# Wenlin-Chen/ADKF-IFT

Hardware: AMD Instinct MI355X
Metric: meta-tasks/sec (N_support=128, d=256) (higher is better)
Workload: dtype f32

## Files before the change

adkf_ift_amd/csrc/adkf_gp.hip:

```cpp
#include <hip/hip_runtime.h>
#include <algorithm>
#include <cstdio>
#include <cstdlib>

#include "../../include/adkf_gp.h"
#include "ard.h"
#include "pna.h"
#include "readout.h"
#include "block.h"
#include "outer_step.h"
#include "refine64.h"
#include "hyper.h"
#include "large_fused.h"
#include "gemm_x3.h"
#include "dense_x3.h"
#include "predict_stream.h"
#include "thompson_stream.h"
#include "believer_stream.h"

#include "host_common.h"
#include "host_gp.h"
#include "host_ard.h"
#include "host_stream.h"

extern "C" {

const char* adkf_last_hip_error(void) { return hipGetErrorString(g_last_hip_error); }

const char* adkf_version(void) { return "adkf_gp 0.1 (gfx950)"; }

int adkf_path_info(int32_t ns_max, int32_t nq_max) {
    if (ns_max <= 0 || nq_max < 0 || ns_max > MAX_POINTS || nq_max > MAX_POINTS) return ADKF_E_SIZE;
    int bits = 0;
    const int hi = ns_max > nq_max ? ns_max : nq_max;
    if (nq_max > 0 && use_fused_outer(ns_max, nq_max)) bits |= ADKF_PATH_FUSED_OUTER;
    if (hi > REG_POINTS) { bits |= ADKF_PATH_BLOCKED; if (lg_fused_by_size(hi)) bits |= ADKF_PATH_BLOCKED_FUSED; }
    if (carve(nullptr, 1, ns_max, nq_max > 0 ? nq_max : 1, 4).w64_stride != 0) bits |= ADKF_PATH_R64_REGION;
    if (refine64_lds_optin()) bits |= ADKF_PATH_R64_LDS;
    return bits;
}

int adkf_max_points(void) { return MAX_POINTS; }

size_t adkf_workspace_bytes(int32_t T, int32_t ns_max, int32_t nq_max, int32_t d) {
    if (T <= 0 || ns_max <= 0 || nq_max < 0 || d <= 0) return 0;
    return carve(nullptr, T, ns_max, nq_max, d).bytes;
}

size_t adkf_workspace_bytes_ard(int32_t T, int32_t ns_max, int32_t nq_max, int32_t d) {
    if (T <= 0 || ns_max <= 0 || nq_max < 0 || d <= 0) return 0;
    return carve_ard(nullptr, carve(nullptr, T, ns_max, nq_max, d).bytes, T, ns_max, nq_max, d).bytes;
}

static int median_core(const adkf_batch_t* b, const Workspace& w, float* l0, const InitArgs& init, bool* fused, hipStream_t st) {
    int rc = stage_dist(b, w, has_query(b), st);
    if (rc) return rc;
    *fused = b->ns_max <= 256;
    if (b->ns_max <= 128) k_median<512, 16><<<grid_for(b->T, 1), 512, 0, st>>>(w.D2ss, b->n_s, b->ns_max, l0, b->T, init);
    else if (b->ns_max <= 256) k_median<1024, 32><<<grid_for(b->T, 1), 1024, 0, st>>>(w.D2ss, b->n_s, b->ns_max, l0, b->T, init);
    else {
        LgMedian lm{w.D2ss, b->n_s, b->ns_max, l0, b->T, reinterpret_cast<uint32_t*>(w.lg_med), w.lg_med + b->T, w.lg_med + 2 * (size_t)b->T};
        hipMemsetAsync(lm.hist, 0, sizeof(int) * 256 * (size_t)b->T, st);
        const int rows_blocks = ceil_div(b->ns_max, 16) < 64 ? ceil_div(b->ns_max, 16) : 64;
        for (int pass = 0; pass < 4; ++pass) {
            k_lg_med_hist<<<dim3(rows_blocks, b->T), 256, 0, st>>>(lm, pass);
            k_lg_med_pick<<<ceil_div(b->T, 64), 64, 0, st>>>(lm, pass);
        }
    }
    LAUNCH_OK();
    return 0;
}

int adkf_median_lengthscale(const adkf_batch_t* b, float* l0, void* ws, size_t ws_bytes, void* stream) {
    int rc = check_batch(b, false);
    if (rc) return rc;
    if (!l0 || !ws) return ADKF_E_BADARG;
    Workspace w = carve_for(b, ws);
    if (ws_bytes < w.bytes) return ADKF_E_WORKSPACE;
    bool fused;
    return median_core(b, w, l0, InitArgs{0, 0, nullptr, nullptr}, &fused, static_cast<hipStream_t>(stream));
}

int adkf_init_params(const adkf_batch_t* b, int32_t use_numeric_labels, int32_t use_lengthscale_prior, float* phi,
                     float* priors, float* l0, void* ws, size_t ws_bytes, void* stream) {
    int rc = check_batch(b, false);
    if (rc) return rc;
    if (!phi || !priors || !ws) return ADKF_E_BADARG;
    Workspace w = carve_for(b, ws);
    if (ws_bytes < w.bytes) return ADKF_E_WORKSPACE;
    float* l0p = l0 ? l0 : w.l0;
    hipStream_t st = static_cast<hipStream_t>(stream);
    InitArgs init{use_numeric_labels, use_lengthscale_prior, phi, priors};
    ArdWs a{};
    if (is_ard(b)) {
        a = carve_ard(ws, w.bytes, b->T, b->ns_max, b->nq_max, b->d);
        if (ws_bytes < a.bytes) return ADKF_E_WORKSPACE;
        init.phi = a.phi3;
    }
    bool fused = false;
    rc = median_core(b, w, l0p, init, &fused, st);
    if (rc) return rc;
    if (!fused) k_init_params<<<ceil_div(b->T, 64), 64, 0, st>>>(l0p, b->T, init);
    if (is_ard(b)) k_ard_expand_phi<<<dim3(ceil_div(2 + b->d, 256), b->T), 256, 0, st>>>(a.phi3, phi, b->T, 2 + b->d);
    LAUNCH_OK();
    return 0;
}

int adkf_mll_value_grad(const adkf_batch_t* b, const float* phi, float* f_in, float* g_phi, float* dZ_s, int32_t* info,
                        void* ws, size_t ws_bytes, void* stream) {
    int rc = check_batch(b, false);
    if (rc) return rc;
    if (!phi || !f_in || !info || !ws || !b->y_s || !b->priors) return ADKF_E_BADARG;
    if (is_ard(b)) {
        ArdCtx c;
        adkf_batch_t b0 = *b; b0.flags &= ~ADKF_BATCH_REUSE_INNER;
        rc = ard_setup(&b0, ws, ws_bytes, static_cast<hipStream_t>(stream), c);
        if (rc) return rc;
        rc = ard_eval(c, phi, f_in, g_phi ? g_phi : c.a.ge, info);
        if (rc) return rc;
        if (dZ_s) {
            ArdDzFin fs{c.v, c.a.G, nullptr, nullptr, nullptr, 0.f, dZ_s, b->n_s, c.ns};
            k_ard_dz_fin<<<dim3(ceil_div(c.d, 256), c.ns, c.T), 256, 0, c.st>>>(fs);
            LAUNCH_OK();
        }
        return 0;
    }
    Workspace w = carve_for(b, ws);
    if (ws_bytes < w.bytes) return ADKF_E_WORKSPACE;
    hipStream_t st = static_cast<hipStream_t>(stream);
    rc = stage_dist(b, w, has_query(b), st);
    if (rc) return rc;
    InnerArgs ia = inner_args(b, w, const_cast<float*>(phi), info);
    ia.f_out = f_in; ia.g_out = g_phi;
    rc = launch_inner(ia, w, st);
    if (rc) return rc;
    launch_refine(make_tv(b, w, false), b, w, false, 0, nullptr, info, st, f_in, g_phi, nullptr);
    if (dZ_s) {
        TaskView tv = make_tv(b, w, false);
        const int win_tiles = std::max(1, std::min(64, b->ns_max * b->ns_max / 2048));
        WinArgs wa{tv, w.Ainv, w.D2ss, w.Wss, w.scal, b->T, win_tiles};
        k_win<<<grid_for(b->T, win_tiles), 256, 0, st>>>(wa);
        hipMemsetAsync(dZ_s, 0, (size_t)b->T * b->ns_max * b->d * sizeof(float), st);
        ProbDZ<false> pz; pz.tv = tv; pz.Wss = w.Wss; pz.Wqs = nullptr; pz.Wqq = nullptr; pz.Zs = b->Z_s; pz.Zq = nullptr; pz.dZ = dZ_s; pz.d = b->d;
        launch_gemm(pz, b->T, b->ns_max, b->d, st, x3_for(b->d));
        LAUNCH_OK();
    }
    return 0;
}

int adkf_fit(const adkf_batch_t* b, float* phi, const adkf_fit_options_t* opt, float* f_final, float* gnorm,
             int32_t* n_evals, int32_t* info, void* ws, size_t ws_bytes, void* stream) {
    int rc = check_batch(b, false);
    if (rc) return rc;
    if (!phi || !opt || !info || !ws || !b->y_s || !b->priors || opt->max_evals < 2) return ADKF_E_BADARG;
    if (is_ard(b)) return ard_fit(b, phi, opt, f_final, gnorm, n_evals, info, ws, ws_bytes, static_cast<hipStream_t>(stream));
    Workspace w = carve_for(b, ws);
    if (ws_bytes < w.bytes) return ADKF_E_WORKSPACE;
    hipStream_t st = static_cast<hipStream_t>(stream);
    rc = stage_dist(b, w, has_query(b), st);
    if (rc) return rc;
    InnerArgs ia = inner_args(b, w, phi, info);
    ia.f_out = f_final; ia.gnorm_out = gnorm; ia.nevals_out = n_evals;
    ia.max_evals = opt->max_evals; ia.exact_evals = opt->exact_evals; ia.gtol = opt->gtol; ia.ftol = opt->ftol;
    if (opt->ev_start && hipEventRecord(static_cast<hipEvent_t>(opt->ev_start), st) != hipSuccess) return ADKF_E_LAUNCH;
    rc = launch_inner(ia, w, st);
    if (opt->ev_stop && hipEventRecord(static_cast<hipEvent_t>(opt->ev_stop), st) != hipSuccess) return ADKF_E_LAUNCH;
    if (rc) return rc;
    if (!(b->flags & ADKF_BATCH_DEFER_REFINE)) launch_refine(make_tv(b, w, false), b, w, false, 0, nullptr, info, st, f_final, nullptr, gnorm);
    LAUNCH_OK();
    return 0;
}

int adkf_predict(const adkf_batch_t* b, const float* phi, float* mean, float* var, float* cov, int32_t* info, void* ws,
                 size_t ws_bytes, void* stream) {
    int rc = check_batch(b, true);
    if (rc) return rc;
    if (!phi || !mean || !info || !ws || !b->y_s || !b->priors) return ADKF_E_BADARG;
    if (is_ard(b)) {
        ArdCtx c;
        rc = ard_setup(b, ws, ws_bytes, static_cast<hipStream_t>(stream), c);
        if (rc) return rc;
        if (b->flags & ADKF_BATCH_REUSE_INNER) k_ard_params<<<dim3(ceil_div(c.d, 256), c.T), 256, 0, c.st>>>(c.v, phi);
        rc = ard_outer(c, phi, 0, nullptr, info, false);
        if (rc) return rc;
        adkf_batch_t bq = c.bt;
        return predict_core(&bq, c.w, mean, var, cov, info, c.st);
    }
    Workspace w = carve_for(b, ws);
    if (ws_bytes < w.bytes) return ADKF_E_WORKSPACE;
    hipStream_t st = static_cast<hipStream_t>(stream);
    rc = stage_dist(b, w, true, st);
    if (rc) return rc;
    rc = inner_stage(b, w, phi, info, true, st);
    if (rc) return rc;
    return predict_core(b, w, mean, var, cov, info, st);
}

int adkf_predict_marginal(const adkf_batch_t* b, const float* phi, int32_t flags, const float* Zq, const int64_t* q_off, int64_t rows,
                          const float* best_f, float* mean, float* var, float* ei, int32_t* info, void* ws, size_t ws_bytes, void* stream) {
    return predict_marginal(false, b, phi, flags, Zq, q_off, rows, best_f, mean, var, ei, info, ws, ws_bytes, stream);
}

int adkf_predict_marginal_ard(const adkf_batch_t* b, const float* phi, int32_t flags, const float* Zq, const int64_t* q_off, int64_t rows,
                              const float* best_f, float* mean, float* var, float* ei, int32_t* info, void* ws, size_t ws_bytes, void* stream) {
    return predict_marginal(true, b, phi, flags, Zq, q_off, rows, best_f, mean, var, ei, info, ws, ws_bytes, stream);
}

size_t adkf_predict_pool_scratch_bytes(int32_t T, int32_t k) {
    if (T <= 0 || k <= 0 || k > ADKF_POOL_TOPK_MAX) return 0;
    return pool_scratch(nullptr, T, k).bytes;
}

int adkf_predict_pool(const adkf_batch_t* b, const float* phi, int32_t flags, const float* X, int64_t rows, const float* best_f,
                      const int64_t* excl_idx, const int64_t* excl_off, float* mean, float* var, float* ei, int32_t k, int64_t* top_idx,
                      float* top_val, int32_t* info, void* ws, size_t ws_bytes, void* scratch, size_t scratch_bytes, void* stream) {
    int rc = check_support_only(b, phi, info, ws, rows);
    if (rc) return rc;
    if (k < 0) return ADKF_E_BADARG;
    if (flags & ~(ADKF_PM_LATENT | ADKF_PM_MAXIMIZE | ADKF_PM_SCORE_MEAN | ADKF_PM_LOG_EI)) return ADKF_E_BADARG;
    const bool by_mean = (flags & ADKF_PM_SCORE_MEAN) != 0;
    if ((flags & ADKF_PM_LOG_EI) && !ei && (k == 0 || by_mean)) return ADKF_E_BADARG;
    if (rows > 0 && !X) return ADKF_E_BADARG;
    if ((ei || (k > 0 && !by_mean)) && !best_f) return ADKF_E_BADARG;
    if (k > 0 && (!top_idx || !top_val)) return ADKF_E_BADARG;
    if (!mean && !var && !ei && k == 0) return ADKF_E_BADARG;
    if (excl_idx && !excl_off) return ADKF_E_BADARG;
    if (k > ADKF_POOL_TOPK_MAX) return ADKF_E_SIZE;
    const PoolScratch l = pool_scratch(scratch, b->T, k);
    if ((rc = check_scratch(scratch, scratch_bytes, l.bytes))) return rc;
    PmCtx c;
    rc = pm_prepare(b, phi, info, ws, ws_bytes, stream, c);
    if (rc) return rc;
    PmPool pool = pm_pool(excl_idx, excl_off, k, b->T, l.cand_idx, l.cand_val, rows, c.st);
    pool.score_mean = by_mean ? 1 : 0; pool.top_idx = top_idx; pool.top_val = top_val;
    const PmCall io{flags & (ADKF_PM_LATENT | ADKF_PM_MAXIMIZE | ADKF_PM_LOG_EI), X, nullptr, rows, best_f, mean, var, ei, info, &pool};
    return c.ard ? pm_launch<true, true>(c, io) : pm_launch<false, true>(c, io);
}

size_t adkf_thompson_pool_scratch_bytes(int32_t T, int32_t ns_max, int32_t S, int32_t m) {
    if (T <= 0 || ns_max <= 0 || ns_max > MAX_POINTS || S < 1 || S > ADKF_TS_SAMPLES_MAX) return 0;
    if (m < 64 || m > ADKF_TS_FEATURES_MAX || (m & 63)) return 0;
    return ts_scratch(nullptr, T, ns_max, S).bytes;
}

int adkf_thompson_pool(const adkf_batch_t* b, const float* phi, int32_t flags, const float* X, int64_t rows, const float* omega,
                       const float* phase, int32_t m, const float* w, const float* eps, int32_t S, const int64_t* excl_idx,
                       const int64_t* excl_off, float* paths, int64_t* sel_idx, float* sel_val, int32_t* info, void* ws, size_t ws_bytes,
                       void* scratch, size_t scratch_bytes, void* stream) {
    return thompson_pool(false, b, phi, flags, X, rows, omega, phase, m, w, eps, S, excl_idx, excl_off, paths, sel_idx, sel_val, info, ws,
                         ws_bytes, scratch, scratch_bytes, stream);
}

int adkf_thompson_pool_ard(const adkf_batch_t* b, const float* phi, int32_t flags, const float* X, int64_t rows, const float* omega,
                           const float* phase, int32_t m, const float* w, const float* eps, int32_t S, const int64_t* excl_idx,
                           const int64_t* excl_off, float* paths, int64_t* sel_idx, float* sel_val, int32_t* info, void* ws, size_t ws_bytes,
                           void* scratch, size_t scratch_bytes, void* stream) {
    return thompson_pool(true, b, phi, flags, X, rows, omega, phase, m, w, eps, S, excl_idx, excl_off, paths, sel_idx, sel_val, info, ws,
                         ws_bytes, scratch, scratch_bytes, stream);
}

size_t adkf_believer_pool_scratch_bytes(int32_t T, int32_t ns_max, int32_t d, int32_t q) {
    if (T <= 0 || ns_max <= 0 || ns_max > MAX_POINTS || d <= 0 || q < 1 || q > ADKF_POOL_TOPK_MAX) return 0;
    return bv_scratch(nullptr, T, ns_max, d, q).bytes;
}

int adkf_believer_pool(const adkf_batch_t* b, const float* phi, int32_t flags, const float* X, int64_t rows, const float* best_f,
                       const int64_t* excl_idx, const int64_t* excl_off, int32_t q, float* trace, int64_t* sel_idx, float* sel_val,
                       float* sel_mean, float* sel_var, int32_t* info, void* ws, size_t ws_bytes, void* scratch, size_t scratch_bytes,
                       void* stream) {
    return believer_pool(false, b, phi, flags, X, rows, best_f, excl_idx, excl_off, q, trace, sel_idx, sel_val, sel_mean, sel_var, info, ws,
                         ws_bytes, scratch, scratch_bytes, stream);
}

int adkf_believer_pool_ard(const adkf_batch_t* b, const float* phi, int32_t flags, const float* X, int64_t rows, const float* best_f,
                           const int64_t* excl_idx, const int64_t* excl_off, int32_t q, float* trace, int64_t* sel_idx, float* sel_val,
                           float* sel_mean, float* sel_var, int32_t* info, void* ws, size_t ws_bytes, void* scratch, size_t scratch_bytes,
                           void* stream) {
    return believer_pool(true, b, phi, flags, X, rows, best_f, excl_idx, excl_off, q, trace, sel_idx, sel_val, sel_mean, sel_var, info, ws,
                         ws_bytes, scratch, scratch_bytes, stream);
}

int adkf_outer_nll_value_grad(const adkf_batch_t* b, const float* phi, float* f_out, float* g_phi, float* dZ_s,
                              float* dZ_q, int32_t* info, void* ws, size_t ws_bytes, void* stream) {
    int rc = check_batch(b, true);
    if (rc) return rc;
    if (!phi || !f_out || !info || !ws || !b->y_s || !b->y_q || !b->priors) return ADKF_E_BADARG;
    if (is_ard(b))
        return ard_ift(b, phi, 0, false, 0, 0.f, f_out, dZ_s, dZ_q, g_phi, nullptr, nullptr, info, ws, ws_bytes, static_cast<hipStream_t>(stream));
    Workspace w = carve_for(b, ws);
    if (ws_bytes < w.bytes) return ADKF_E_WORKSPACE;
    return outer_pipeline(b, w, phi, 0, false, f_out, dZ_s, dZ_q, g_phi, nullptr, nullptr, info, static_cast<hipStream_t>(stream));
}

int adkf_ift_hypergrad(const adkf_batch_t* b, const float* phi, int32_t flags, float* f_out, float* dZ_s, float* dZ_q,
                       float* g_phi_out, float* v, float* H, int32_t* info, void* ws, size_t ws_bytes, void* stream) {
    int rc = check_batch(b, true);
    if (rc) return rc;
    if (!phi || !f_out || !dZ_s || !dZ_q || !info || !ws || !b->y_s || !b->y_q || !b->priors) return ADKF_E_BADARG;
    if (is_ard(b)) {
        if (H) return ADKF_E_BADARG;
        return ard_ift(b, phi, flags, true, ADKF_CG_DEFAULT_MAXITER, ADKF_CG_DEFAULT_TOL, f_out, dZ_s, dZ_q, g_phi_out, v, nullptr, info,
                       ws, ws_bytes, static_cast<hipStream_t>(stream));
    }
    Workspace w = carve_for(b, ws);
    if (ws_bytes < w.bytes) return ADKF_E_WORKSPACE;
    return outer_pipeline(b, w, phi, flags, true, f_out, dZ_s, dZ_q, g_phi_out, v, H, info, static_cast<hipStream_t>(stream));
}

int adkf_double_path_tasks(const adkf_batch_t* b, int32_t* flagged, void* ws, size_t ws_bytes, void* stream) {
    int rc = check_batch(b, true);
    if (rc) return rc;
    if (!flagged || !ws || is_ard(b)) return ADKF_E_BADARG;
    Workspace w = carve_for(b, ws);
    if (ws_bytes < w.bytes) return ADKF_E_WORKSPACE;
    (void)hipGetLastError();
    k_double_path_tasks<<<ceil_div(b->T, 256), 256, 0, static_cast<hipStream_t>(stream)>>>(w.scal, b->ns_max, b->nq_max, w.w64 ? r64_threshold() : INFINITY, b->T, flagged);
    LAUNCH_OK();
    return 0;
}

int adkf_ift_hypergrad_cg(const adkf_batch_t* b, const float* phi, int32_t flags, int32_t cg_maxiter, float cg_tol, float* f_out,
                          float* dZ_s, float* dZ_q, float* g_phi_out, float* v, int32_t* cg_iters, int32_t* info, void* ws,
                          size_t ws_bytes, void* stream) {
    int rc = check_batch(b, true);
    if (rc) return rc;
    if (!is_ard(b) || cg_maxiter < 1 || !(cg_tol > 0.f)) return ADKF_E_BADARG;
    if (!phi || !f_out || !dZ_s || !dZ_q || !info || !ws || !b->y_s || !b->y_q || !b->priors) return ADKF_E_BADARG;
    return ard_ift(b, phi, flags, true, cg_maxiter, cg_tol, f_out, dZ_s, dZ_q, g_phi_out, v, cg_iters, info, ws, ws_bytes,
                   static_cast<hipStream_t>(stream));
}

int adkf_check_info(const int32_t* info, int32_t T, void* stream) {
    if (!info || T <= 0) return ADKF_E_BADARG;
    int32_t* host = static_cast<int32_t*>(malloc(sizeof(int32_t) * (size_t)T));
    if (!host) return ADKF_E_BADARG;
    hipStream_t st = static_cast<hipStream_t>(stream);
    if (hipMemcpyAsync(host, info, sizeof(int32_t) * (size_t)T, hipMemcpyDeviceToHost, st) != hipSuccess || hipStreamSynchronize(st) != hipSuccess) {
        free(host);
        return ADKF_E_LAUNCH;
    }
    int rc = 0;
    for (int t = 0; t < T; ++t) if (host[t] != 0) { rc = t + 1; break; }
    free(host);
    return rc;
}

}

#include "host_gnn.h"
#include "host_dense.h"
```

adkf_ift_amd/csrc/host_gp.h:

```cpp
#pragma once
#include "host_common.h"

namespace {

inline bool x3_for(int d) { return d >= GK; }

struct Workspace {
    float *mean, *D2ss, *D2qs, *D2qq, *Ainv, *P, *C, *S, *OC, *Wss, *Wqs, *Wqq, *vecs, *scal, *part_oc, *part_ma, *l0;
    float *lg_Dinv, *lg_C, *lg_F, *lg_logdet, *lg_part, *lg_pext;
    int32_t *lg_info, *lg_med, *lg_cnt;
    FitShared* lg_fit;
    double* w64; size_t w64_stride;
    int vld, nt_oc, nt_ma;
    int lg_mode;
    size_t bytes;
};

Workspace carve(void* base, int T, int ns, int nq, int d) {
    Workspace w{};
    Arena ar{static_cast<char*>(base), 0};
    const size_t Tz = (size_t)T;
    w.vld = ns > nq ? ns : nq;
    w.nt_oc = nq > 0 ? tiles_of(nq, ns) : 0;
    w.nt_ma = tiles_of(ns, ns);
    w.mean = ar.floats(Tz * d);
    w.D2ss = ar.floats(Tz * ns * ns);
    w.D2qs = ar.floats(Tz * nq * ns);
    w.D2qq = ar.floats(Tz * nq * nq);
    w.Ainv = ar.floats(Tz * ns * ns);
    w.P = ar.floats(Tz * ns * ns);
    w.C = ar.floats(Tz * nq * ns);
    w.S = ar.floats(Tz * nq * nq);
    w.OC = ar.floats(Tz * nq * ns);
    w.Wss = ar.floats(Tz * ns * ns);
    w.Wqs = ar.floats(Tz * nq * ns);
    w.Wqq = ar.floats(Tz * nq * nq);
    w.vecs = ar.floats(Tz * NVEC * w.vld);
    w.scal = ar.floats(Tz * NSCAL);
    w.part_oc = ar.floats(Tz * (w.nt_oc > 0 ? w.nt_oc : 1) * 4);
    w.part_ma = ar.floats(Tz * w.nt_ma * 4);
    w.l0 = ar.floats(Tz);
    if (w.vld > REG_POINTS) {
        w.lg_Dinv = ar.floats(2 * Tz * LB * LB);
        w.lg_C = ar.floats(Tz * LB * w.vld);
        w.lg_F = ar.floats(Tz * LB * w.vld);
        w.lg_logdet = ar.floats(Tz);
        w.lg_pext = ar.floats(Tz * 2);
        const size_t tq = (size_t)((nq + GT - 1) / GT) * ((nq + GT - 1) / GT);
        const size_t ts = (size_t)((ns + GT - 1) / GT) * ((ns + GT - 1) / GT);
        w.lg_part = ar.floats(Tz * (ts > tq ? ts : tq) * 8);
        w.lg_info = ar.as<int32_t>(Tz);
        w.lg_cnt = ar.as<int32_t>(Tz);
        w.lg_med = ar.as<int32_t>(Tz * 258);
        static_assert(sizeof(FitShared) % sizeof(float) == 0, "FitShared is carved as whole floats");
        w.lg_fit = ar.as<FitShared>(Tz);
    }
    if (w.vld <= r64_maxn()) {
        w.w64_stride = refine64_doubles(ns, nq);
        w.w64 = ar.as<double>(Tz * w.w64_stride);
    }
    w.bytes = ar.off;
    return w;
}

Workspace carve_for(const adkf_batch_t* b, void* ws) {
    Workspace w = carve(ws, b->T, b->ns_max, b->nq_max, b->d);
    w.lg_mode = (b->flags & ADKF_BATCH_LG_UNFUSED) ? -1 : (b->flags & ADKF_BATCH_LG_FUSED) ? 1 : 0;
    return w;
}

int check_batch(const adkf_batch_t* b, bool need_query) {
    (void)hipGetLastError();
    if (!b || b->T <= 0 || b->ns_max <= 0 || b->d <= 0 || !b->Z_s) return ADKF_E_BADARG;
    if (b->kernel != ADKF_KERNEL_RBF && b->kernel != ADKF_KERNEL_MATERN52) return ADKF_E_BADARG;
    if (b->ns_max > MAX_POINTS) return ADKF_E_SIZE;
    if (need_query) {
        if (b->nq_max <= 0 || !b->Z_q) return ADKF_E_BADARG;
        if (b->nq_max > MAX_POINTS) return ADKF_E_SIZE;
    }
    return 0;
}

bool vec_ok(const adkf_batch_t* b, const Workspace& w) {
    if ((b->ns_max & 3) || (b->nq_max & 3) || (b->d & 3) || (w.vld & 3)) return false;
    return aligned16(b->Z_s) && aligned16(b->Z_q) && aligned16(w.mean);
}

TaskView make_tv(const adkf_batch_t* b, const Workspace& w, bool with_query) {
    TaskView tv;
    tv.n_s = b->n_s; tv.n_q = with_query ? b->n_q : nullptr;
    tv.ns_ld = b->ns_max; tv.nq_ld = with_query ? b->nq_max : 0; tv.vld = w.vld; tv.kind = b->kernel;
    tv.scal = w.scal; tv.vecs = w.vecs;
    tv.vec = vec_ok(b, w);
    return tv;
}

inline bool has_query(const adkf_batch_t* b) { return b->nq_max > 0 && b->Z_q != nullptr; }
inline bool is_ard(const adkf_batch_t* b) { return (b->flags & ADKF_BATCH_ARD) != 0; }

int stage_dist(const adkf_batch_t* b, const Workspace& w, bool with_query, hipStream_t st, int parts = 3) {
    if (b->flags & ADKF_BATCH_REUSE_DIST) return 0;
    const int T = b->T, ns = b->ns_max, nq = with_query ? b->nq_max : 0, d = b->d;
    if (!(parts & 2)) with_query = false;
    if ((parts & 1) && !(parts & 4)) k_colmean<<<dim3(ceil_div(d, 64), T), 256, 0, st>>>(b->Z_s, b->n_s, ns, d, w.mean, T);
    ProbDist p;
    p.mean = w.mean; p.d = d; p.vec = vec_ok(b, w);
    ProbDistMulti pm;
    pm.vec = p.vec; pm.end0 = pm.end1 = 0; pm.tn0 = pm.tn1 = pm.tn2 = 1;
    int nblk = 0, total = 0;
    auto add = [&](const ProbDist& q, int M, int N) {
        const int tn = ceil_div(N, GT), tiles = ceil_div(M, GT) * tn;
        if (nblk == 0) { pm.s0 = q; pm.tn0 = tn; pm.end0 = pm.end1 = total + tiles; pm.s1 = pm.s2 = q; }
        else if (nblk == 1) { pm.s1 = q; pm.tn1 = tn; pm.end1 = total + tiles; pm.s2 = q; }
        else { pm.s2 = q; pm.tn2 = tn; }
        total += tiles; ++nblk;
    };
    if (parts & 1) {
        p.X = b->Z_s; p.Y = b->Z_s; p.n_x = b->n_s; p.n_y = b->n_s; p.x_ld = ns; p.y_ld = ns; p.symmetric = true; p.D2 = w.D2ss;
        add(p, ns, ns);
    }
    if (with_query) {
        p.X = b->Z_q; p.Y = b->Z_s; p.n_x = b->n_q; p.n_y = b->n_s; p.x_ld = nq; p.y_ld = ns; p.symmetric = false; p.D2 = w.D2qs;
        add(p, nq, ns);
        p.X = b->Z_q; p.Y = b->Z_q; p.n_x = b->n_q; p.n_y = b->n_q; p.x_ld = nq; p.y_ld = nq; p.symmetric = true; p.D2 = w.D2qq;
        add(p, nq, nq);
    }
    if (nblk > 0) {
        if (x3_for(d)) k_bgemm3<ProbDistMulti, GT, 256><<<grid_for(T, total), 256, 0, st>>>(pm, T, 1, total);
        else k_bgemm<ProbDistMulti, GT><<<grid_for(T, total), 256, 0, st>>>(pm, T, 1, total);
    }
    LAUNCH_OK();
    return 0;
}

template <int NMAX, int NT, bool LOW>
void launch_inner_kl(const InnerArgs& a, hipStream_t st) {
    constexpr size_t cache_bytes = sizeof(float) * NMAX * NMAX;
    static const bool optin = lds_optin(cache_bytes, {kernel_ptr(&k_inner<NMAX, NT, 0, LOW>), kernel_ptr(&k_inner<NMAX, NT, 1, LOW>)});
    (void)optin;
    if (a.kind == ADKF_KERNEL_RBF) k_inner<NMAX, NT, 0, LOW><<<grid_for(a.T, 1), NT, cache_bytes, st>>>(a);
    else k_inner<NMAX, NT, 1, LOW><<<grid_for(a.T, 1), NT, cache_bytes, st>>>(a);
}

template <int NMAX, int NT>
void launch_inner_k(const InnerArgs& a, hipStream_t st) {
    if constexpr (NMAX == 128) {
        if (a.T > num_cus()) { launch_inner_kl<NMAX, NT, true>(a, st); return; }
    }
    launch_inner_kl<NMAX, NT, false>(a, st);
}

inline bool lg_fused_by_size(int ld) { return ld >= 4 * LB; }

LgMat lg_mat(const Workspace& w, float* M, int ld, const int32_t* n_arr, const FitShared* fit, int T) {
    LgMat m;
    m.M = M; m.ld = ld; m.n_arr = n_arr; m.fit = fit;
    m.Dinv = w.lg_Dinv; m.Cbuf = w.lg_C; m.Fbuf = w.lg_F; m.logdet = w.lg_logdet; m.pext = w.lg_pext; m.info = w.lg_info;
    const bool fused = w.lg_mode > 0 || (w.lg_mode == 0 && lg_fused_by_size(ld));
    m.cnt = fused ? w.lg_cnt : nullptr;
    m.T = T; m.vec = (ld & 3) == 0;
    return m;
}

void lg_sweep(const LgMat& m0, hipStream_t st) {
    const int nb = ceil_div(m0.ld, LB), tn = ceil_div(m0.ld, GT);
    LgMat m = m0;
    if (m.cnt) {
        float* dinv[2] = {m0.Dinv, m0.Dinv + (size_t)m0.T * LB * LB};
        const int npair = lgf_npair(tn);
        k_lg_diag<<<grid_for(m.T, 1), 512, 0, st>>>(m, 0);
        for (int step = 0; step < nb; ++step) {
            m.Dinv = dinv[step & 1];
            ProbLgPanel pp; pp.m = m; pp.step = step;
            k_bgemm<ProbLgPanel><<<grid_for(m.T, 2 * tn), 256, 0, st>>>(pp, m.T, 2, tn);
            LgStepArgs sa{m, dinv[(step + 1) & 1], m.cnt, step, tn, npair, step + 1 < nb ? 1 : 0};
            k_lg_update_sweep<<<grid_for(m.T, npair), LGF_NT, 0, st>>>(sa);
        }
        return;
    }
    for (int step = 0; step < nb; ++step) {
        k_lg_diag<<<grid_for(m.T, 1), 512, 0, st>>>(m, step);
        ProbLgPanel pp; pp.m = m; pp.step = step;
        k_bgemm<ProbLgPanel><<<grid_for(m.T, 2 * tn), 256, 0, st>>>(pp, m.T, 2, tn);
        ProbLgUpdate pu; pu.m = m; pu.step = step; pu.tri = tn * (tn + 1) / 2;
        k_bgemm<ProbLgUpdate><<<grid_for(m.T, pu.tri), 256, 0, st>>>(pu, m.T, tn, tn);
    }
}

constexpr int POLL_EVERY = 8;

__global__ void k_count_unfinished(const char* base, size_t stride, size_t phase_offset, int T, int done_value, int32_t* out) {
    int c = 0;
    for (int t = threadIdx.x; t < T; t += blockDim.x) c += *reinterpret_cast<const int*>(base + (size_t)t * stride + phase_offset) != done_value;
    c = wave_sum_i(c);
    if (threadIdx.x == 0) *out = c;
}

struct FitPoll {
    bool enabled = false;
    int32_t* host = nullptr;
    int32_t* dev;
    FitPoll(bool convergence_mode, int max_evals, int32_t* dev_counter, hipStream_t st) : dev(dev_counter) {
        if (!convergence_mode || max_evals <= 2 * POLL_EVERY) return;
        hipStreamCaptureStatus cs = hipStreamCaptureStatusNone;
        if (hipStreamIsCapturing(st, &cs) != hipSuccess || cs != hipStreamCaptureStatusNone) return;
        thread_local int32_t* pinned = nullptr;
        if (!pinned && hipHostMalloc(reinterpret_cast<void**>(&pinned), sizeof(int32_t), hipHostMallocDefault) != hipSuccess) return;
        host = pinned;
        enabled = true;
    }
    bool finished(int e, const void* state, size_t stride, size_t phase_offset, int T, hipStream_t st, int done_value = PH_DONE, int every_after = POLL_EVERY) {
        if (!enabled) return false;
        if (e + 1 < POLL_EVERY || (e + 1 - POLL_EVERY) % every_after != 0) return false;
        k_count_unfinished<<<1, 64, 0, st>>>(static_cast<const char*>(state), stride, phase_offset, T, done_value, dev);
        if (hipMemcpyAsync(host, dev, sizeof(int32_t), hipMemcpyDeviceToHost, st) != hipSuccess) return false;
        if (hipStreamSynchronize(st) != hipSuccess) return false;
        return *host == 0;
    }
};

int launch_inner_large(const InnerArgs& a, const Workspace& w, hipStream_t st) {
    LgInner li;
    li.in = a; li.fit = w.lg_fit; li.part = w.lg_part;
    li.tiles_1d = ceil_div(a.ld, GT); li.ntiles = li.tiles_1d * li.tiles_1d;
    li.mat = lg_mat(w, a.Ainv, a.ld, a.n_s, w.lg_fit, a.T);
    LgMatvecArgs mv{li.mat, a.y_s, (size_t)a.ld, a.vecs + (size_t)V_ALPHA * a.vld, (size_t)NVEC * a.vld, -1.f};
    k_lg_begin<<<ceil_div(a.T, 64), 64, 0, st>>>(li);
    const int n_evals = a.max_evals > 0 ? a.max_evals : 1;
    FitPoll poll(a.max_evals > 0 && !a.exact_evals, a.max_evals, w.lg_info, st);
    for (int e = 0; e < n_evals; ++e) {
        k_lg_build<<<grid_for(a.T, li.ntiles), 256, 0, st>>>(li);
        lg_sweep(li.mat, st);
        k_lg_matvec<<<dim3(ceil_div(a.ld, 4), a.T), 256, 0, st>>>(mv);
        k_lg_traces<<<grid_for(a.T, li.ntiles), 256, 0, st>>>(li);
        k_lg_advance<<<a.T, 256, 0, st>>>(li);
        if (poll.finished(e, w.lg_fit, sizeof(FitShared), offsetof(FitShared, phase), a.T, st)) break;
    }
    LAUNCH_OK();
    return 0;
}

int launch_inner(InnerArgs a, const Workspace& w, hipStream_t st) {
    if (a.ld > REG_POINTS) return launch_inner_large(a, w, st);
    if (a.ld <= 16) launch_inner_k<16, 256>(a, st);
    else if (a.ld <= 32) launch_inner_k<32, 256>(a, st);
    else if (a.ld <= 64) launch_inner_k<64, 256>(a, st);
    else launch_inner_k<128, 512>(a, st);
    LAUNCH_OK();
    return 0;
}

void launch_alpha_refine(const TaskView& tv, const adkf_batch_t* b, const Workspace& w, hipStream_t st) {
    AlphaRefineArgs aa{tv, w.Ainv, w.D2ss, b->y_s, w.vecs, refine32_threshold(), b->T};
    k_alpha_refine<<<grid_for(b->T, 1), SMALL_NT, 0, st>>>(aa);
}

void launch_c(const TaskView& tv, const adkf_batch_t* b, const Workspace& w, hipStream_t st) {
    const int T = b->T, ns = b->ns_max, nq = b->nq_max;
    ProbC pc; pc.tv = tv; pc.Ainv = w.Ainv; pc.D2qs = w.D2qs; pc.C = w.C;
    launch_gemm(pc, T, nq, ns, st);
    ProbCres pr; pr.tv = tv; pr.C = w.C; pr.D2ss = w.D2ss; pr.D2qs = w.D2qs; pr.R = w.OC; pr.thresh = refine32_threshold();
    launch_gemm(pr, T, nq, ns, st);
    ProbCfix pf; pf.tv = tv; pf.R = w.OC; pf.Ainv = w.Ainv; pf.C = w.C; pf.thresh = refine32_threshold();
    launch_gemm(pf, T, nq, ns, st);
}

bool refine64_lds_optin() {
    static const bool ok = lds_optin(sizeof(double) * R64_LDS_POINTS * R64_LDS_POINTS, {kernel_ptr(&k_refine64), kernel_ptr(&k_tail64)});
    return ok;
}

Refine64Args refine_args(const TaskView& tv, const adkf_batch_t* b, const Workspace& w, bool with_hessian, int level, float* f_out,
                         int32_t* info, float* f_in, float* g_in, float* gnorm, size_t& lds_bytes) {
    const bool lds_inv = refine64_lds_optin();
    lds_bytes = lds_inv ? sizeof(double) * (size_t)R64_LDS_POINTS * R64_LDS_POINTS : 0;
    return Refine64Args{tv, b->Z_s, b->Z_q, b->d, b->y_s, b->y_q, b->priors, w.Ainv, with_hessian ? w.P : nullptr, level >= 1 ? w.C : nullptr,
                        level >= 2 ? w.S : nullptr, w.vecs, w.scal, f_out, info, f_in, g_in, gnorm, w.w64, w.w64_stride, r64_threshold(), b->T,
                        with_hessian ? 1 : 0, level, lds_inv ? 1 : 0};
}

void launch_refine(const TaskView& tv, const adkf_batch_t* b, const Workspace& w, bool with_hessian, int level, float* f_out,
                   int32_t* info, hipStream_t st, float* f_in = nullptr, float* g_in = nullptr, float* gnorm = nullptr) {
    if (!w.w64) return;
    size_t lds_bytes;
    const Refine64Args ra = refine_args(tv, b, w, with_hessian, level, f_out, info, f_in, g_in, gnorm, lds_bytes);
    k_refine64<<<b->T, R64_NT, lds_bytes, st>>>(ra);
}

bool use_fused_outer(int ns, int nq) {
    static const bool optin = lds_optin(HY_LDS_BYTES, {kernel_ptr(&k_hyper<true, 0>), kernel_ptr(&k_hyper<true, 1>),
                                                       kernel_ptr(&k_hyper<false, 0>), kernel_ptr(&k_hyper<false, 1>)});
    const int hi = ns > nq ? ns : nq;
    return optin && hi >= 1 && hi <= HY_N;
}

int launch_outer_factor(const OuterArgs& a, const Workspace& w, int nq, hipStream_t st) {
    if (nq > REG_POINTS) {
        k_lg_resid<<<dim3(ceil_div(nq, 4), a.T), 256, 0, st>>>(a);
        LgMat m = lg_mat(w, a.S, a.tv.nq_ld, a.tv.n_q, nullptr, a.T);
        lg_sweep(m, st);
        LgMatvecArgs mv{m, a.vecs + (size_t)V_R * a.tv.vld, (size_t)NVEC * a.tv.vld, a.vecs + (size_t)V_E * a.tv.vld, (size_t)NVEC * a.tv.vld, -1.f};
        k_lg_matvec<<<dim3(ceil_div(nq, 4), a.T), 256, 0, st>>>(mv);
        const int tn = ceil_div(nq, GT);
        k_lg_negate<<<grid_for(a.T, tn * tn), 256, 0, st>>>(m, tn);
        LgColsumArgs cs{a.C, a.tv.ns_ld, (size_t)a.tv.nq_ld * a.tv.ns_ld, a.tv.n_q, a.tv.nq_ld, a.tv.n_s, a.tv.ns_ld,
                        a.vecs + (size_t)V_E * a.tv.vld, (size_t)NVEC * a.tv.vld, a.vecs + (size_t)V_CTE * a.tv.vld, (size_t)NVEC * a.tv.vld};
        k_lg_colsum<<<dim3(ceil_div(a.tv.ns_ld, 64), a.T), 1024, 0, st>>>(cs);
        LgOuterFin fin{a, w.lg_logdet, w.lg_info, w.lg_pext};
        k_lg_outer_fin<<<a.T, 64, 0, st>>>(fin);
        LAUNCH_OK();
        return 0;
    }
    if (nq <= 16) k_outer_factor<16, 256><<<grid_for(a.T, 1), 256, 0, st>>>(a);
    else if (nq <= 32) k_outer_factor<32, 256><<<grid_for(a.T, 1), 256, 0, st>>>(a);
    else if (nq <= 64) k_outer_factor<64, 256><<<grid_for(a.T, 1), 256, 0, st>>>(a);
    else k_outer_factor<128, 512><<<grid_for(a.T, 1), 512, 0, st>>>(a);
    LAUNCH_OK();
    return 0;
}


InnerArgs inner_args(const adkf_batch_t* b, const Workspace& w, float* phi, int32_t* info) {
    InnerArgs a{};
    a.D2ss = w.D2ss; a.y_s = b->y_s; a.n_s = b->n_s; a.phi = phi; a.priors = b->priors;
    a.Ainv = w.Ainv; a.vecs = w.vecs; a.scal = w.scal; a.info = info;
    a.T = b->T; a.ld = b->ns_max; a.vld = w.vld; a.kind = b->kernel;
    a.max_evals = 0; a.exact_evals = 0; a.gtol = 0.f; a.ftol = 0.f;
    return a;
}

int inner_stage(const adkf_batch_t* b, const Workspace& w, const float* phi, int32_t* info, bool zero_info_on_reuse, hipStream_t st) {
    if (!(b->flags & ADKF_BATCH_REUSE_INNER)) return launch_inner(inner_args(b, w, const_cast<float*>(phi), info), w, st);
    if (zero_info_on_reuse) hipMemsetAsync(info, 0, sizeof(int32_t) * (size_t)b->T, st);
    return 0;
}

int outer_pipeline(const adkf_batch_t* b, const Workspace& w, const float* phi, int flags, bool with_hessian, float* f_out,
                   float* dZ_s, float* dZ_q, float* g_phi_out, float* v_out, float* H_out, int32_t* info, hipStream_t st) {
    const int T = b->T, ns = b->ns_max, nq = b->nq_max, d = b->d;
    int rc = stage_dist(b, w, true, st);
    if (rc) return rc;
    const bool reuse_inner = (b->flags & ADKF_BATCH_REUSE_INNER) != 0;
    rc = inner_stage(b, w, phi, info, false, st);
    if (rc) return rc;
    TaskView tv = make_tv(b, w, true);
    const int tms = ceil_div(ns, GT), tmq = ceil_div(nq, GT);
    const float dirscale = (flags & ADKF_IGNORE_DIRECT_GRAD) ? 0.f : 1.f;
    const float corrscale = (with_hessian && !(flags & ADKF_IGNORE_GRAD_CORRECTION)) ? 1.f : 0.f;
    if (use_fused_outer(ns, nq)) {
        HyperArgs ha{tv, w.Ainv, w.D2ss, w.D2qs, w.D2qq, b->y_s, b->y_q, b->priors, w.Wss, w.Wqs, w.Wqq, w.vecs, w.scal, f_out, info,
                     g_phi_out, v_out, H_out, T, reuse_inner ? 1 : 0, with_hessian ? 1 : 0, flags, dirscale, corrscale, refine32_threshold()};
        const bool full = ns == HY_N && nq == HY_N && !b->n_s && !b->n_q && tv.vec;
        const bool rbf = b->kernel == ADKF_KERNEL_RBF;
        if (full && rbf) k_hyper<true, 0><<<grid_for(T, 1), HY_NT, HY_LDS_BYTES, st>>>(ha);
        else if (full) k_hyper<true, 1><<<grid_for(T, 1), HY_NT, HY_LDS_BYTES, st>>>(ha);
        else if (rbf) k_hyper<false, 0><<<grid_for(T, 1), HY_NT, HY_LDS_BYTES, st>>>(ha);
        else k_hyper<false, 1><<<grid_for(T, 1), HY_NT, HY_LDS_BYTES, st>>>(ha);
    } else {
    launch_alpha_refine(tv, b, w, st);
    if (with_hessian) {
        ProbP pp; pp.tv = tv; pp.Ainv = w.Ainv; pp.D2ss = w.D2ss; pp.P = w.P;
        launch_gemm(pp, T, ns, ns, st);
        HessArgs ha{tv, w.Ainv, w.P, w.D2ss, b->y_s, b->priors, w.scal, w.vecs, T};
        if (ns > REG_POINTS) {
            k_lg_hess_mv<<<dim3(ceil_div(ns, 4), T), 256, 0, st>>>(ha);
            LgMat am = lg_mat(w, w.Ainv, ns, b->n_s, nullptr, T);
            LgMatvecArgs mv{am, w.vecs + (size_t)V_BETA * w.vld, (size_t)NVEC * w.vld, w.vecs + (size_t)V_DELTA * w.vld, (size_t)NVEC * w.vld, 1.f};
            k_lg_matvec<<<dim3(ceil_div(ns, 4), T), 256, 0, st>>>(mv);
            LgHessTr ht{ha, w.lg_part, tms * tms, tms};
            k_lg_hess_tr<<<grid_for(T, tms * tms), 256, 0, st>>>(ht);
            k_lg_hess_fin<<<T, 64, 0, st>>>(ht);
        } else {
            k_hess<<<grid_for(T, 1), SMALL_NT, 0, st>>>(ha);
        }
    }
    launch_c(tv, b, w, st);
    ProbS ps; ps.tv = tv; ps.C = w.C; ps.D2qs = w.D2qs; ps.D2qq = w.D2qq; ps.S = w.S;
    launch_gemm(ps, T, nq, nq, st);
    OuterArgs oa{tv, w.C, w.S, b->y_s, b->y_q, w.vecs, w.scal, f_out, info, T, reuse_inner ? 1 : 0};
    rc = launch_outer_factor(oa, w, nq, st);
    if (rc) return rc;
    ProbOC po; po.tv = tv; po.Sinv = w.S; po.C = w.C; po.D2qs = w.D2qs; po.OC = w.OC; po.Wqs = w.Wqs; po.part = w.part_oc; po.ntiles = w.nt_oc; po.dirscale = dirscale;
    launch_gemm(po, T, nq, ns, st);
    ProbMA pm; pm.tv = tv; pm.C = w.C; pm.OC = w.OC; pm.D2ss = w.D2ss; pm.Wss = w.Wss; pm.part = w.part_ma; pm.ntiles = w.nt_ma; pm.dirscale = dirscale;
    launch_gemm(pm, T, ns, ns, st);
    SolveArgs sa{tv, w.scal, w.vecs, w.part_oc, w.part_ma, w.nt_oc, w.nt_ma, flags, g_phi_out, v_out, H_out, T, with_hessian ? 1 : 0};
    WqqArgs wq{tv, w.S, w.D2qq, w.Wqq, w.scal, dirscale, T, 0, sa};
    if (nq > REG_POINTS) {
        LgWqq lw{wq, w.lg_part, tmq * tmq, tmq};
        k_lg_wqq<<<grid_for(T, tmq * tmq), 256, 0, st>>>(lw);
        k_lg_wqq_fin<<<T, 64, 0, st>>>(lw);
        k_solve_v<<<T, 64, 0, st>>>(sa);
    } else {
        wq.do_solve = 1;
        k_wqq<<<grid_for(T, 1), SMALL_NT, 0, st>>>(wq);
    }
    if (corrscale != 0.f) {
        ProbMixed px; px.tv = tv; px.Ainv = w.Ainv; px.P = w.P; px.D2ss = w.D2ss; px.Wss = w.Wss; px.corrscale = corrscale;
        launch_gemm(px, T, ns, ns, st);
    }
    }
    if (dZ_s || dZ_q) {
        if (dZ_s && b->n_s) hipMemsetAsync(dZ_s, 0, (size_t)T * ns * d * sizeof(float), st);
        if (dZ_q && b->n_q) hipMemsetAsync(dZ_q, 0, (size_t)T * nq * d * sizeof(float), st);
        ProbDZ<false> pzs; pzs.tv = tv; pzs.Wss = w.Wss; pzs.Wqs = w.Wqs; pzs.Wqq = w.Wqq; pzs.Zs = b->Z_s; pzs.Zq = b->Z_q; pzs.dZ = dZ_s; pzs.d = d;
        ProbDZ<true> pzq; pzq.tv = tv; pzq.Wss = w.Wss; pzq.Wqs = w.Wqs; pzq.Wqq = w.Wqq; pzq.Zs = b->Z_s; pzq.Zq = b->Z_q; pzq.dZ = dZ_q; pzq.d = d;
        if (dZ_s) launch_gemm(pzs, T, ns, d, st, x3_for(d));
        if (dZ_q) launch_gemm(pzq, T, nq, d, st, x3_for(d));
    }
    if (w.w64) {
        size_t lds_bytes;
        const Refine64Args ra = refine_args(tv, b, w, with_hessian, 2, f_out, info, nullptr, nullptr, nullptr, lds_bytes);
        Cot64Args ca{tv, b->Z_s, b->Z_q, dZ_s, dZ_q, d, w.vecs, w.scal, w.w64, w.w64_stride, r64_threshold(), T,
                     with_hessian ? 1 : 0, flags, dirscale, corrscale, g_phi_out, v_out, H_out, lds_bytes ? 1 : 0};
        k_tail64<<<T, R64_NT, lds_bytes, st>>>(ra, ca);
    }
    LAUNCH_OK();
    return 0;
}

int predict_core(const adkf_batch_t* b, const Workspace& w, float* mean, float* var, float* cov, int32_t* info, hipStream_t st) {
    TaskView tv = make_tv(b, w, true);
    const int T = b->T;
    launch_alpha_refine(tv, b, w, st);
    launch_c(tv, b, w, st);
    launch_refine(tv, b, w, false, 1, nullptr, info, st);
    PredArgs pa{tv, w.C, w.D2qs, b->y_s, mean, var, w.scal, T};
    k_predict<<<grid_for(T, 1), 256, 0, st>>>(pa);
    if (cov) {
        hipMemsetAsync(cov, 0, (size_t)T * b->nq_max * b->nq_max * sizeof(float), st);
        ProbS ps; ps.tv = tv; ps.C = w.C; ps.D2qs = w.D2qs; ps.D2qq = w.D2qq; ps.S = cov;
        launch_gemm(ps, T, b->nq_max, b->nq_max, st);
    }
    LAUNCH_OK();
    return 0;
}

}
```

Baseline: 291,900.

## Add per-task fused distance kernel computing support/query distance matrices with bf16x3 MFMA

Adds a specialized kernel that, for 128-point support and query sets, computes the support-support, query-support and query-query squared-distance matrices in one workgroup per task. It stages centred inputs as split bf16 operands in double-buffered LDS with prefetching, accumulates with MFMA, and writes symmetric outputs directly. This replaces the generic tiled multi-problem distance launch and is meant to cut launch count and redundant loads of the support set. It applies only when sizes are exactly 128, no per-task counts are given, and the LDS opt-in succeeds.

After: 296,500 (median of 6 runs). 1.02x the previous value.

```diff
diff --git a/adkf_ift_amd/csrc/adkf_gp.hip b/adkf_ift_amd/csrc/adkf_gp.hip
--- a/adkf_ift_amd/csrc/adkf_gp.hip
+++ b/adkf_ift_amd/csrc/adkf_gp.hip
@@ -14,6 +14,7 @@
 #include "large_fused.h"
 #include "gemm_x3.h"
 #include "dense_x3.h"
+#include "dist_task.h"
 #include "predict_stream.h"
 #include "thompson_stream.h"
 #include "believer_stream.h"
diff --git a/adkf_ift_amd/csrc/dist_task.h b/adkf_ift_amd/csrc/dist_task.h
--- /dev/null
+++ b/adkf_ift_amd/csrc/dist_task.h
@@ -0,0 +1,204 @@
+#pragma once
+#include "kernels.h"
+#include "gemm_x3.h"
+
+namespace adkf {
+
+constexpr int DT_N = 128, DT_NT = 512, DT_PLANE = DT_N * X3_RS, DT_OPER = 3 * DT_PLANE, DT_BUF = 2 * DT_OPER;
+constexpr int DT_LDS_BYTES = 2 * DT_BUF * (int)sizeof(unsigned short);
+
+struct DistTaskArgs {
+    const float *Zs, *Zq, *mean;
+    float *D2ss, *D2qs, *D2qq;
+    int d, T;
+};
+
+extern __shared__ __attribute__((aligned(16))) unsigned short dt_lds[];
+
+__global__ __launch_bounds__(DT_NT) void k_dist_task(DistTaskArgs a) {
+    constexpr int MI = 4, MJ = 2, IH = 1;
+    int t, tile;
+    if (!task_tile(a.T, 1, t, tile)) return;
+    __shared__ float rowsq[2][DT_N];
+    const int tid = threadIdx.x, lane = tid & 63, wv = tid >> 6;
+    const int wr = wv >> 2, wc = (wv & 3) ^ (wr << 1), fi = lane & 15, fk = lane >> 4;
+    const int d = a.d, nc = d / GK, last = nc - 1;
+    const bool sym_on = !(wr == 1 && wc < 2);
+
+    const int sr = tid >> 3, sk = (tid & 7) * 4;
+    const char* const zs = reinterpret_cast<const char*>(a.Zs + (size_t)t * DT_N * d);
+    const char* const zq = reinterpret_cast<const char*>(a.Zq + (size_t)t * DT_N * d);
+    const char* const mu = reinterpret_cast<const char*>(a.mean + (size_t)t * d);
+    const size_t hi = (size_t)256 * d;
+    const uint32_t off = 4u * (uint32_t)(sr * d + sk), off_mu = 4u * (uint32_t)sk;
+    auto ldb = [](const char* base, uint32_t o) __attribute__((always_inline)) { return *reinterpret_cast<const float4*>(base + o); };
+    const int frag_a = (wr * 64 + fi) * X3_RS + 8 * fk, frag_b = (wc * 32 + fi) * X3_RS + 8 * fk;
+
+    float4 rs[2][2], rq[2][2], rm;
+    float sqs[2] = {0.f, 0.f}, sqq[2] = {0.f, 0.f};
+    auto fetch = [&](auto with_s, int set, int c) __attribute__((always_inline)) {
+        const size_t k = (size_t)(4 * GK) * c;
+        if constexpr (decltype(with_s)::value) { rs[set][0] = ldb(zs + k, off); rs[set][1] = ldb(zs + hi + k, off); }
+        rq[set][0] = ldb(zq + k, off); rq[set][1] = ldb(zq + hi + k, off);
+    };
+    auto fetch_mean = [&](int c) __attribute__((always_inline)) { rm = ldb(mu + (size_t)(4 * GK) * c, off_mu); };
+    auto centre = [](const float4& r, const float4& m, float (&v)[4]) __attribute__((always_inline)) {
+        constexpr int DPP_IDENTITY = 0xE4;
+        v[0] = dpp_f<DPP_IDENTITY>(r.x) - m.x; v[1] = dpp_f<DPP_IDENTITY>(r.y) - m.y;
+        v[2] = dpp_f<DPP_IDENTITY>(r.z) - m.z; v[3] = dpp_f<DPP_IDENTITY>(r.w) - m.w;
+    };
+    auto stage = [&](auto with_s, int buf, int set, bool commit) __attribute__((always_inline)) {
+        constexpr bool S = decltype(with_s)::value;
+        unsigned short* B = dt_lds + buf * DT_BUF;
+        float v[2][4], ts[2] = {sqs[0], sqs[1]}, tq[2] = {sqq[0], sqq[1]};
+        if constexpr (S) {
+            centre(rs[set][0], rm, v[0]); centre(rs[set][1], rm, v[1]);
+            x3_stage<true, DT_N, DT_NT, 1>(B, v, ts);
+        }
+        centre(rq[set][0], rm, v[0]); centre(rq[set][1], rm, v[1]);
+        x3_stage<true, DT_N, DT_NT, S ? 1 : 0>(B + DT_OPER, v, tq);
+        if constexpr (S) {
+#pragma unroll
+            for (int ps = 0; ps < 2; ++ps) { sqs[ps] = commit ? ts[ps] : sqs[ps]; sqq[ps] = commit ? tq[ps] : sqq[ps]; }
+        }
+    };
+
+    auto block_terms = [&](const unsigned short* Ab, const unsigned short* Bb, const bf16x8 (&b)[2][MJ], f32x4 (&acc)[MI][MJ], f32x4 (&small)[MI][MJ]) __attribute__((always_inline)) {
+#define ADKF_DT_LOADA(dst_, q_) _Pragma("unroll") for (int i = 0; i < IH; ++i) dst_[i] = *reinterpret_cast<const bf16x8*>(Ab + (q_) * DT_PLANE + (ih + i) * 16 * X3_RS);
+#define ADKF_DT_TERM(dst_, av_, bq_)                                                                       \
+    _Pragma("unroll") for (int i = 0; i < IH; ++i) _Pragma("unroll") for (int j = 0; j < MJ; ++j)        \
+        dst_[ih + i][j] = __builtin_amdgcn_mfma_f32_16x16x32_bf16(bq_[j], av_[i], dst_[ih + i][j], 0, 0, 0);
+#pragma unroll
+        for (int ih = 0; ih < MI; ih += IH) {
+            bf16x8 a0[IH], ax[IH], b2[MJ];
+#pragma unroll
+            for (int j = 0; j < MJ; ++j) b2[j] = *reinterpret_cast<const bf16x8*>(Bb + 2 * DT_PLANE + j * 16 * X3_RS);
+            ADKF_DT_LOADA(a0, 0) ADKF_DT_TERM(small, a0, b2)
+            ADKF_DT_LOADA(ax, 2) ADKF_DT_TERM(small, ax, b[0])
+            ADKF_DT_LOADA(ax, 1) ADKF_DT_TERM(small, ax, b[1])
+            ADKF_DT_TERM(acc, a0, b[0])
+            ADKF_DT_TERM(small, a0, b[1]) ADKF_DT_TERM(small, ax, b[0])
+        }
+#undef ADKF_DT_TERM
+#undef ADKF_DT_LOADA
+    };
+    auto load_b = [&](const unsigned short* Bb, bf16x8 (&b)[2][MJ]) __attribute__((always_inline)) {
+#pragma unroll
+        for (int q = 0; q < 2; ++q)
+#pragma unroll
+            for (int j = 0; j < MJ; ++j) b[q][j] = *reinterpret_cast<const bf16x8*>(Bb + q * DT_PLANE + j * 16 * X3_RS);
+    };
+    auto run_pass = [&](auto with_s, auto&& multiply) __attribute__((always_inline)) {
+        auto advance = [&](int c, int nbuf, int nset, bool commit) __attribute__((always_inline)) {
+            stage(with_s, nbuf, nset, commit);
+            fetch_mean(min(c + 2, last));
+            __builtin_amdgcn_sched_barrier(0);
+            fetch(with_s, nset, min(c + 3, last));
+        };
+        stage(with_s, 0, 0, true);
+        fetch_mean(min(1, last));
+        __builtin_amdgcn_sched_barrier(0);
+        fetch(with_s, 0, min(2, last));
+        __syncthreads();
+        int c = 0;
+        for (; c + 1 < nc; c += 2) {
+            multiply(0); advance(c, 1, 1, true); __syncthreads();
+            multiply(1); advance(c + 1, 0, 0, c + 2 < nc); __syncthreads();
+        }
+        if (c < nc) { multiply(0); __syncthreads(); }
+    };
+    auto zero = [](f32x4 (&x)[MI][MJ]) __attribute__((always_inline)) {
+#pragma unroll
+        for (int i = 0; i < MI; ++i)
+#pragma unroll
+            for (int j = 0; j < MJ; ++j) x[i][j] = (f32x4){0.f, 0.f, 0.f, 0.f};
+    };
+    auto values = [&](const f32x4& acc, const float* nrow, const float* ncol, int gi, int gj0, float (&v)[4]) __attribute__((always_inline)) {
+        const float nx = nrow[gi];
+        const float4 ny = *reinterpret_cast<const float4*>(ncol + gj0);
+        v[0] = fmaxf(nx + ny.x - 2.f * acc[0], 0.f); v[1] = fmaxf(nx + ny.y - 2.f * acc[1], 0.f);
+        v[2] = fmaxf(nx + ny.z - 2.f * acc[2], 0.f); v[3] = fmaxf(nx + ny.w - 2.f * acc[3], 0.f);
+    };
+    auto store_sym = [&](float* D, const f32x4& acc, const float* nrm, int rt, int ct) __attribute__((always_inline)) {
+        const int gi = rt * 16 + fi, gj0 = ct * 16 + fk * 4;
+        float v[4];
+        values(acc, nrm, nrm, gi, gj0, v);
+        if (rt < ct) {
+            *reinterpret_cast<float4*>(D + (size_t)gi * DT_N + gj0) = make_float4(v[0], v[1], v[2], v[3]);
+#pragma unroll
+            for (int r = 0; r < 4; ++r) D[(size_t)(gj0 + r) * DT_N + gi] = v[r];
+        } else {
+#pragma unroll
+            for (int r = 0; r < 4; ++r) {
+                const int gj = gj0 + r;
+                if (gi == gj) D[(size_t)gi * DT_N + gj] = 0.f;
+                else if (gi < gj) { D[(size_t)gi * DT_N + gj] = v[r]; D[(size_t)gj * DT_N + gi] = v[r]; }
+            }
+        }
+    };
+
+    const std::true_type pass1{};
+    const std::false_type pass2{};
+    float* const Dss = a.D2ss + (size_t)t * DT_N * DT_N;
+    float* const Dqs = a.D2qs + (size_t)t * DT_N * DT_N;
+    float* const Dqq = a.D2qq + (size_t)t * DT_N * DT_N;
+
+    fetch_mean(0);
+    __builtin_amdgcn_sched_barrier(0);
+    fetch(pass1, 0, 0); fetch(pass1, 1, min(1, last));
+    {
+        f32x4 acc_s[MI][MJ], small_s[MI][MJ], acc_q[MI][MJ], small_q[MI][MJ];
+        zero(acc_s); zero(small_s); zero(acc_q); zero(small_q);
+        run_pass(pass1, [&](int buf) __attribute__((always_inline)) {
+            const unsigned short* S = dt_lds + buf * DT_BUF;
+            bf16x8 b[2][MJ];
+            load_b(S + frag_b, b);
+            if (sym_on) block_terms(S + frag_a, S + frag_b, b, acc_s, small_s);
+            __builtin_amdgcn_sched_barrier(0);
+            block_terms(S + DT_OPER + frag_a, S + frag_b, b, acc_q, small_q);
+        });
+        fetch_mean(0);
+        __builtin_amdgcn_sched_barrier(0);
+        fetch(pass2, 0, 0); fetch(pass2, 1, min(1, last));
+#pragma unroll
+        for (int ps = 0; ps < 2; ++ps) {
+            float s = sqs[ps], q = sqq[ps];
+            s += dpp_f<DPP_XOR1>(s); s += dpp_f<DPP_XOR2>(s); s += dpp_f<DPP_HALF_MIRROR>(s);
+            q += dpp_f<DPP_XOR1>(q); q += dpp_f<DPP_XOR2>(q); q += dpp_f<DPP_HALF_MIRROR>(q);
+            if ((tid & 7) == 0) { rowsq[0][sr + ps * 64] = s; rowsq[1][sr + ps * 64] = q; }
+        }
+        __syncthreads();
+#pragma unroll
+        for (int i = 0; i < MI; ++i)
+#pragma unroll
+            for (int j = 0; j < MJ; ++j) {
+                const int rt = wr * 4 + i, ct = wc * 2 + j;
+                float v[4];
+                values(acc_q[i][j] + small_q[i][j], rowsq[1], rowsq[0], rt * 16 + fi, ct * 16 + fk * 4, v);
+                *reinterpret_cast<float4*>(Dqs + (size_t)(rt * 16 + fi) * DT_N + ct * 16 + fk * 4) = make_float4(v[0], v[1], v[2], v[3]);
+                if (rt <= ct) store_sym(Dss, acc_s[i][j] + small_s[i][j], rowsq[0], rt, ct);
+            }
+    }
+
+    {
+        f32x4 acc_g[MI][MJ], small_g[MI][MJ];
+        zero(acc_g); zero(small_g);
+        run_pass(pass2, [&](int buf) __attribute__((always_inline)) {
+            if (sym_on) {
+                const unsigned short* Q = dt_lds + buf * DT_BUF + DT_OPER;
+                bf16x8 b[2][MJ];
+                load_b(Q + frag_b, b);
+                block_terms(Q + frag_a, Q + frag_b, b, acc_g, small_g);
+            }
+        });
+#pragma unroll
+        for (int i = 0; i < MI; ++i)
+#pragma unroll
+            for (int j = 0; j < MJ; ++j) {
+                const int rt = wr * 4 + i, ct = wc * 2 + j;
+                if (rt <= ct) store_sym(Dqq, acc_g[i][j] + small_g[i][j], rowsq[1], rt, ct);
+            }
+    }
+}
+
+}
diff --git a/adkf_ift_amd/csrc/host_gp.h b/adkf_ift_amd/csrc/host_gp.h
--- a/adkf_ift_amd/csrc/host_gp.h
+++ b/adkf_ift_amd/csrc/host_gp.h
@@ -98,11 +98,22 @@
 inline bool has_query(const adkf_batch_t* b) { return b->nq_max > 0 && b->Z_q != nullptr; }
 inline bool is_ard(const adkf_batch_t* b) { return (b->flags & ADKF_BATCH_ARD) != 0; }
 
+bool use_dist_task(const adkf_batch_t* b, const Workspace& w, bool with_query, int parts) {
+    static const bool optin = lds_optin(DT_LDS_BYTES, {kernel_ptr(&k_dist_task)});
+    return optin && parts == 3 && with_query && b->ns_max == DT_N && b->nq_max == DT_N && !b->n_s && !b->n_q && (b->d % GK) == 0 &&
+           b->d <= (1 << 22) && vec_ok(b, w);
+}
+
 int stage_dist(const adkf_batch_t* b, const Workspace& w, bool with_query, hipStream_t st, int parts = 3) {
     if (b->flags & ADKF_BATCH_REUSE_DIST) return 0;
     const int T = b->T, ns = b->ns_max, nq = with_query ? b->nq_max : 0, d = b->d;
     if (!(parts & 2)) with_query = false;
     if ((parts & 1) && !(parts & 4)) k_colmean<<<dim3(ceil_div(d, 64), T), 256, 0, st>>>(b->Z_s, b->n_s, ns, d, w.mean, T);
+    if (use_dist_task(b, w, with_query, parts)) {
+        k_dist_task<<<grid_for(T, 1), DT_NT, DT_LDS_BYTES, st>>>(DistTaskArgs{b->Z_s, b->Z_q, w.mean, w.D2ss, w.D2qs, w.D2qq, d, T});
+        LAUNCH_OK();
+        return 0;
+    }
     ProbDist p;
     p.mean = w.mean; p.d = d; p.vec = vec_ok(b, w);
     ProbDistMulti pm;
```
